# ToniChopp/ECAMP

Hardware: AMD Instinct MI355X
Metric: pretrain image-report pairs/sec (ViT-B/16, 224^2, seq=128) (higher is better)
Workload: dtype bf16

## Files before the change

ecamp_amd/csrc/core.hip:

```cpp
#include "common.h"
#include "attention.h"
#include "options.h"
#include "../../include/ecamp_hip.h"
#include <atomic>
#include <stdarg.h>
#include <stdlib.h>

thread_local char g_ecamp_err[512] = {0};

int ecamp_set_error(int code, const char* fmt, ...) {
    va_list ap;
    va_start(ap, fmt);
    vsnprintf(g_ecamp_err, sizeof(g_ecamp_err), fmt, ap);
    va_end(ap);
    return code;
}

extern "C" const char* ecamp_last_error(void) { return g_ecamp_err; }
extern "C" int ecamp_abi_version(void) { return ECAMP_ABI_VERSION; }
extern "C" int ecamp_half_format(void) { return ECAMP_HALF_IS_F16; }

#define OPT_UNREAD (INT_MIN + 1)
struct OptRow {
    const char* name; const char* env; int def; int (*set)(int);
    std::atomic<int> value{OPT_ENV};
    std::atomic<int> env_value{OPT_UNREAD};
};
static OptRow g_opts[OPT_COUNT] = {
              {"q8_mode", "ECAMP_GEMM_Q8", -1, [](int v) { return v == 0 || v == 2 ? v : -1; }},
               {"q8_sch", "ECAMP_Q8_SCH", 7, [](int v) { return v >= 0 ? v : OPT_ENV; }},
             {"q16_mode", "ECAMP_Q16", 1, [](int v) { return v >= 0 && v <= 3 ? v : OPT_ENV; }},
                {nullptr, "ECAMP_F8_Q8", 1, nullptr},
         {nullptr, "ECAMP_Q8_MIN_ITEMS", OPT_AUTO, nullptr},
          {"q8_bwd_grid", "ECAMP_Q8_BWD_GRID", 0, [](int v) { return v > 0 ? v : OPT_ENV; }},
             {"p8_wgrad", nullptr, 1, [](int v) { return v ? 1 : 0; }},
     {"p8_wgrad_reserve_cus", nullptr, 0, [](int v) { return v < 0 ? 0 : v; }},
          {nullptr, "ECAMP_WGRAD_ITEMS", 0, nullptr},
           {nullptr, "ECAMP_WGRAD_PLAN", 1, nullptr},
      {nullptr, "ECAMP_WGRAD_GROUP_CUS", 0, nullptr},
        {nullptr, "ECAMP_GEMM_GRID_CAP", 0, nullptr},
            {"attn_head", "ECAMP_ATTN_HEAD", 1, [](int v) { return v < 0 ? OPT_ENV : v ? 1 : 0; }},
           {nullptr, "ECAMP_ATTN_WAVES", 0, nullptr},
               {nullptr, "ECAMP_LN_BWD", 0, nullptr},
            {nullptr, "ECAMP_CE_KERNEL", 1, nullptr},
            {nullptr, "ECAMP_SR_BLOCKS", 512, nullptr},
};
int ecamp_opt_default(EcampOpt id) { return g_opts[id].def; }
int ecamp_opt(EcampOpt id) {
    OptRow& o = g_opts[id];
    const int s = o.value.load(std::memory_order_relaxed);
    if (s != OPT_ENV) return s;
    int e = o.env_value.load(std::memory_order_relaxed);
    if (e == OPT_UNREAD) {
        const char* txt = o.env ? getenv(o.env) : nullptr;
        e = txt ? atoi(txt) : o.def;
        o.env_value.store(e, std::memory_order_relaxed);
    }
    return e;
}
bool ecamp_opt_set(const char* name, int value) {
    for (OptRow& o : g_opts)
        if (o.name && strcmp(name, o.name) == 0) {
            o.value.store(o.set(value), std::memory_order_relaxed);
            return true;
        }
    return false;
}
extern "C" int ecamp_set_option(const char* name, int32_t value) {
    ECAMP_CHECK_ARG(name != nullptr, "set_option: null name");
    if (strcmp(name, "attn_head") == 0) { attn_set_head_mode(value); return 0; }
    if (ecamp_opt_set(name, value)) return 0;
    return ecamp_set_error(-1, "set_option: unknown option '%s'", name);
}

__global__ void dev_spin_kernel(long long cycles) {
    const long long t0 = clock64();
    while (clock64() - t0 < cycles) {}
}
extern "C" int ecamp_dev_spin(int32_t blocks, int32_t threads, int64_t cycles, hipStream_t stream) {
    ECAMP_CHECK_ARG(blocks > 0 && threads > 0 && threads <= 1024 && cycles >= 0, "dev_spin: bad arguments");
    hipLaunchKernelGGL(dev_spin_kernel, dim3(blocks), dim3(threads), 0, stream, (long long)cycles);
    ECAMP_LAUNCH_CHECK();
    return 0;
}
// ... 1 lines not shown
```

ecamp_amd/csrc/gemm.hip:

```cpp
#include "common.h"
#include <stdlib.h>
#include <string.h>
#include <stdint.h>
#include <map>
#include <string>
#include <vector>

#include "gemm_args.h"
#include "gemm_q8.h"
#include "gemm_q16.h"

#define BM 128
#define BN 128
#define BK 64

__device__ __forceinline__ int swz(int row) { return (row >> 1) & 7; }

__device__ __forceinline__ void g2r_kc(const bf16_t* P, long ld, int row0, int nrows, int k0, int kend, int tid,
                                       uint4 (&r)[4]) {
#pragma unroll
    for (int i = 0; i < 4; ++i) {
        int c = tid + 256 * i;
        int row = c >> 3, kc = c & 7;
        int gr = row0 + row, gk = k0 + kc * 8;
// ... 585 lines not shown
    if (g.out_f32) return (!g.bias && !g.residual && !g.pre_out && !g.gmul && !g.act) ? 4 : -1;
    if (g.gmul) return (!g.bias && !g.pre_out && (g.act == 0 || g.act == 2)) ? 3 : -1;
    if (g.pre_out || g.act) return (g.pre_out && (g.act == 1 || g.act == 2) && !g.residual) ? 1 : -1;
    if (g.residual) return 2;
    return 0;
}
static gemm_fn q8_pick(int a_kc, int b_kc, int epi, bool rowsum) {
    const int sch = ecamp_opt(OPT_Q8_SCH);
#define Q8S(A, B, E, R) ((gemm_fn)gemm_bf16_q8_kernel<A, B, E, 0, R, 1>)
    if (a_kc && b_kc && (sch & 1)) return epi == 0 ? Q8S(true, true, 0, false) : epi == 1 ? Q8S(true, true, 1, false) : epi == 2 ? Q8S(true, true, 2, false) :
                                          epi == 5 ? Q8S(true, true, 5, false) : (gemm_fn) nullptr;
    if (a_kc && !b_kc && (sch & 2)) return epi == 0 ? Q8S(true, false, 0, false) : epi == 2 ? Q8S(true, false, 2, false) : epi == 3 ? Q8S(true, false, 3, false) : (gemm_fn) nullptr;
    if (!a_kc && !b_kc && epi == 4 && (sch & 4)) return rowsum ? Q8S(false, false, 4, true) : Q8S(false, false, 4, false);
#undef Q8S
    if (a_kc && b_kc) return epi == 0 ? gemm_bf16_q8_kernel<true, true, 0> : epi == 1 ? gemm_bf16_q8_kernel<true, true, 1> : epi == 2 ? gemm_bf16_q8_kernel<true, true, 2> : (gemm_fn) nullptr;
    if (a_kc && !b_kc) return epi == 0 ? gemm_bf16_q8_kernel<true, false, 0> : epi == 2 ? gemm_bf16_q8_kernel<true, false, 2> : epi == 3 ? gemm_bf16_q8_kernel<true, false, 3> : (gemm_fn) nullptr;
    if (!a_kc && !b_kc && epi == 4) return rowsum ? gemm_bf16_q8_kernel<false, false, 4, 0, true> : gemm_bf16_q8_kernel<false, false, 4, 0, false>;
    return nullptr;
}
static bool q8_legal(const GemmArgs& g, int a_kc, int b_kc, int dtype, bool res32) {
    if (dtype != ECAMP_BF16) return false;
    const int epi = q8_epi(g, res32), split_k = g.nsplit;
    if (epi < 0 || !q8_pick(a_kc, b_kc, epi, g.rowsum != nullptr)) return false;
    if (split_k > 1 && epi != 4) return false;
    const long M = g.M, N = g.N, K = g.K;
    long kps = (K + split_k - 1) / split_k;
    kps = (kps + 63) / 64 * 64;
    const long ns = (K + kps - 1) / kps, last = K - (ns - 1) * kps;
    if (kps < 128 || last <= 64) return false;
    if (N % 8 || g.lda % 8 || g.ldb % 8 || !al16(g.A) || !al16(g.B) || !al16(g.C)) return false;
    if ((a_kc ? M * g.lda : K * g.lda) * 2 > LIM_2GB || (b_kc ? N * g.ldb : K * g.ldb) * 2 > LIM_2GB) return false;
    if (!a_kc && M % 8) return false;
    if (split_k > 1) { if (!al16(g.partial) || (long)split_k * M * N * 4 > LIM_2GB) return false; }
    else if (g.ldc % 8 || M * g.ldc * (epi >= 4 ? 4 : 2) > LIM_2GB) return false;
    if (g.bias && !al16(g.bias)) return false;
    if (g.pre_out && (g.ldp % 8 || !al16(g.pre_out) || M * g.ldp * 2 > LIM_2GB)) return false;
    if (g.gmul && (g.ldg % 8 || !al16(g.gmul) || M * g.ldg * 2 > LIM_2GB)) return false;
    if (g.residual && (g.ldr % 8 || !al16(g.residual) || M * g.ldr * (res32 ? 4 : 2) > LIM_2GB)) return false;
    return true;
}
static double q16_cost(int64_t M, int64_t N, int tn, int ncu) {
    const long tiles = (long)ceil_div(M, 256) * ceil_div(N, tn);
    return (double)((tiles + ncu - 1) / ncu) * (tn == 192 ? 0.79 : 1.0);
}
static gemm_fn q16_pick(int b_kc, int epi, int nw) {
    if (epi == 5) return b_kc ? (nw == 8 ? (gemm_fn)gemm_bf16_q16_kernel<5, 8, true> : (gemm_fn)gemm_bf16_q16_kernel<5, 6, true>) : (gemm_fn) nullptr;
    if (b_kc) {
        if (nw == 8) return epi == 0 ? (gemm_fn)gemm_bf16_q16_kernel<0, 8, true> : (gemm_fn)gemm_bf16_q16_kernel<2, 8, true>;
        return epi == 0 ? (gemm_fn)gemm_bf16_q16_kernel<0, 6, true> : (gemm_fn)gemm_bf16_q16_kernel<2, 6, true>;
    }
    if (nw == 8) return epi == 0 ? (gemm_fn)gemm_bf16_q16_kernel<0, 8, false> : (gemm_fn)gemm_bf16_q16_kernel<2, 8, false>;
    return epi == 0 ? (gemm_fn)gemm_bf16_q16_kernel<0, 6, false> : (gemm_fn)gemm_bf16_q16_kernel<2, 6, false>;
}

enum GemmFamily { GEMM_T128, GEMM_Q8, GEMM_Q16 };
struct GemmChoice {
    GemmFamily family;
    gemm_fn fn;
    int tm, tn;
    int block;
    long cap;
    const char* name;
    char form, epi, tail;
};
static GemmChoice gemm_select(const GemmArgs& g, int a_kc, int b_kc, int dtype, bool res32) {
    const char form = a_kc && b_kc ? 'f' : a_kc ? 'd' : 'w';
    GemmChoice c = {GEMM_T128, t128_pick(dtype, a_kc, b_kc, g.rowsum != nullptr, res32), BM, BN, 256, 0, "t128", form, '-', 's'};
    const int q8m = ecamp_opt(OPT_Q8_MODE), m16 = ecamp_opt(OPT_Q16_MODE);
    const long items8 = (long)ceil_div(g.M, 256) * ceil_div(g.N, 256) * g.nsplit;
    if (q8m == 0 || !(q8m == 2 || items8 >= q8_min_items() || m16 == 3) || !(a_kc || b_kc || ecamp_opt(OPT_P8_WGRAD)) || !q8_legal(g, a_kc, b_kc, dtype, res32))
        return c;
    const int epi = q8_epi(g, res32), ncu = p8_num_cu();
    c.epi = (char)('0' + epi);
    const int bwd_grid = a_kc && !b_kc ? ecamp_opt(OPT_Q8_BWD_GRID) : 0;
    if (m16 > 0 && a_kc && (epi == 0 || epi == 2 || epi == 5) && g.nsplit == 1 && !g.rowsum && (b_kc || g.ldb % 8 == 0)) {
        const double c256 = q16_cost(g.M, g.N, 256, ncu), c192 = q16_cost(g.M, g.N, 192, ncu);
        const int nw = c192 <= 0.9 * c256 ? 6 : 8;
        if (m16 >= 2 || nw == 6) {
            c.family = GEMM_Q16; c.fn = q16_pick(b_kc, epi, nw); c.tm = 256; c.tn = nw * 32; c.block = 256; c.name = "q16"; c.tail = 'w';
            c.cap = bwd_grid > 0 ? bwd_grid : ncu;
            return c;
        }
    }
    c.family = GEMM_Q8; c.fn = q8_pick(a_kc, b_kc, epi, g.rowsum != nullptr); c.tm = 256; c.tn = 256; c.block = 512; c.name = "q8";
    c.cap = bwd_grid > 0 ? bwd_grid : a_kc && b_kc ? ncu : p8_bwd_cus();
    return c;
}

extern "C" int ecamp_gemm_suggest_split(int64_t M, int64_t N, int64_t K, int a_kc, int b_kc, int dtype) {
    if (M <= 0 || N <= 0 || K <= 0) return 1;
    const int ncu = a_kc && b_kc ? p8_num_cu() : p8_bwd_cus();
    const long tiles = (long)ceil_div(M, 128) * ceil_div(N, 128);
    long s_old = 1024 / tiles;
    if (s_old < 1) s_old = 1;
    const long cap = (K + 255) / 256;
    if (s_old > cap) s_old = cap;
    if (dtype != ECAMP_BF16 || ecamp_opt(OPT_Q8_MODE) == 0 || (a_kc != 0) != (b_kc != 0) || (!a_kc && !b_kc && !ecamp_opt(OPT_P8_WGRAD))) return (int)s_old;
    const long t8 = (long)ceil_div(M, 256) * ceil_div(N, 256);
    const long tgt = (!a_kc && !b_kc) ? wgrad_target_items(ncu) : ncu;
    int best = 1;
    double best_score = -1.0;
    for (int sp = 1; sp <= 32; ++sp) {
        if (sp > 1 && K / sp < 512) break;
        const long items = t8 * sp;
        const long rounds = (items + tgt - 1) / tgt;
        const double score = (double)items / (double)(rounds * tgt) - 0.012 * (sp - 1);
        if (score > best_score + 1e-9) { best_score = score; best = sp; }
    }
    return t8 * best >= q8_min_items() ? best : (int)s_old;
}

extern "C" int64_t ecamp_gemm_workspace_bytes(int64_t M, int64_t N, int64_t K, int32_t split_k) {
    (void)K;
    return split_k > 1 && M > 0 && N > 0 ? (int64_t)split_k * M * N * 4 : 0;
}

static int gemm_call(const void* A, const void* B, void* C, int64_t M, int64_t N, int64_t K, int a_kc, int64_t lda,
                     int b_kc, int64_t ldb, int64_t ldc, const float* bias, const void* residual, int64_t ldr,
                     void* pre_out, int64_t ldp, const void* gmul, int64_t ldg, int act, float alpha, const float* alpha_dev, int dtype,
                     int out_f32, int accumulate, int split_k, float* splitk_ws, float* rowsum, hipStream_t stream, bool res32) {
    ECAMP_CHECK_ARG(A && B && C, "ecamp_gemm: null operand");
    ECAMP_CHECK_ARG(M > 0 && N > 0 && K > 0, "ecamp_gemm: bad shape %ld %ld %ld", (long)M, (long)N, (long)K);
    ECAMP_CHECK_ARG(dtype == ECAMP_F32 || dtype == ECAMP_BF16, "ecamp_gemm: bad dtype %d", dtype);
    ECAMP_CHECK_ARG(act >= 0 && act <= 2, "ecamp_gemm: act=%d (0 none, 1 GELU, 2 GELU with the saved derivative)", act);
    ECAMP_CHECK_ARG(act != 2 || (dtype == ECAMP_BF16 && !out_f32 && ((pre_out != nullptr) != (gmul != nullptr))),
                    "ecamp_gemm: act=2 (saved derivative) is the bf16 forward form with pre_out or the data-gradient form with gmul");
    const int vec = dtype == ECAMP_BF16 ? 8 : 4;
    const int ovec = dtype == ECAMP_BF16 ? 8 : 4;
    ECAMP_CHECK_ARG(N % 4 == 0, "ecamp_gemm: N=%ld must be a multiple of 4", (long)N);
    if (a_kc) ECAMP_CHECK_ARG(K % vec == 0 && lda % vec == 0, "ecamp_gemm: K/lda alignment (A k-contiguous)");
    else ECAMP_CHECK_ARG(M % ovec == 0 && lda % ovec == 0, "ecamp_gemm: M/lda alignment (A m-contiguous), M=%ld", (long)M);
    if (b_kc) ECAMP_CHECK_ARG(K % vec == 0 && ldb % vec == 0, "ecamp_gemm: K/ldb alignment (B k-contiguous)");
    else ECAMP_CHECK_ARG(N % ovec == 0 && ldb % ovec == 0, "ecamp_gemm: N/ldb alignment (B n-contiguous)");
    ECAMP_CHECK_ARG(!accumulate || out_f32 || dtype == ECAMP_F32, "ecamp_gemm: accumulate needs an f32 output");
    ECAMP_CHECK_ARG(!rowsum || (!a_kc && !b_kc), "ecamp_gemm: rowsum is built for the weight-gradient form (both operands strided) only");
// ... 261 lines not shown
extern "C" int64_t ecamp_wgrad_group_table_bytes(int32_t n, const int64_t* n_out, const int64_t* k_in, int64_t rows) {
    if (!ecamp_wgrad_group_supported(n, n_out, k_in, rows)) return 0;
    const long tiles = wg_tiles(n, n_out, k_in), ncu = p8_num_cu();
    return (tiles + ncu + 1) * (long)sizeof(Q8ItemRec) + ((ncu + 2) * 4 + 31) / 32 * 32 + tiles * (long)sizeof(WgTile) + 64;
}
extern "C" int64_t ecamp_wgrad_group_table(int32_t n, const int64_t* n_out, const int64_t* k_in, const int32_t* has_bias, int64_t rows,
                                           int32_t workgroups, void* host_table) {
    if (!n_out || !k_in || !has_bias || !host_table || !ecamp_wgrad_group_supported(n, n_out, k_in, rows))
        return ecamp_set_error(-1, "wgrad_group_table: unsupported group or null pointer");
    unsigned hb[4] = {0, 0, 0, 0};
    for (int p = 0; p < n; ++p) hb[p] = has_bias[p] ? 1u : 0u;
    const WgPlan* pl = wg_plan(n, n_out, k_in, hb, rows, ecamp_wgrad_group_workgroups(workgroups));
    char* out = (char*)host_table;
    memcpy(out, pl->items.data(), pl->items.size() * sizeof(Q8ItemRec));
    memcpy(out + pl->off_first, pl->first.data(), pl->first.size() * sizeof(int));
    memcpy(out + pl->off_tiles, pl->tiles.data(), pl->tiles.size() * sizeof(WgTile));
    return (int64_t)pl->bytes;
}
extern "C" int ecamp_wgrad_group(int32_t n, const void* const* dy, const void* const* x, float* const* gw, float* const* gb, const int64_t* n_out,
                                 const int64_t* k_in, int64_t rows, float alpha, const float* alpha_dev, const int32_t* accumulate, float* ws,
                                 const void* table, int64_t table_bytes, int32_t workgroups, hipStream_t stream) {
    ECAMP_CHECK_ARG(dy && x && gw && gb && n_out && k_in && accumulate && ws && table, "wgrad_group: null pointer");
    ECAMP_CHECK_ARG(((uintptr_t)table & 31) == 0, "wgrad_group: the item table must be 32-byte aligned");
    ECAMP_CHECK_ARG(ecamp_wgrad_group_supported(n, n_out, k_in, rows), "wgrad_group: unsupported group (1-4 layers, rows >= 256, dims %% 8 == 0, < 2 GB operands)");
    unsigned hb[4] = {0, 0, 0, 0};
    bool any_bias = false;
    for (int p = 0; p < n; ++p) {
        ECAMP_CHECK_ARG(dy[p] && x[p] && gw[p], "wgrad_group: null operand");
        ECAMP_CHECK_ARG(((uintptr_t)dy[p] & 15) == 0 && ((uintptr_t)x[p] & 15) == 0 && ((uintptr_t)gw[p] & 15) == 0, "wgrad_group: operands must be 16-byte aligned");
        hb[p] = gb[p] ? 1u : 0u;
        any_bias = any_bias || gb[p];
    }
    const int nwg = ecamp_wgrad_group_workgroups(workgroups);
    const WgPlan* pl = wg_plan(n, n_out, k_in, hb, rows, nwg);
    ECAMP_CHECK_ARG(table_bytes == (int64_t)pl->bytes, "wgrad_group: the item table (%ld bytes) was not built for the current plan (%ld bytes: CU reserve "
                    "or workgroup count changed since ecamp_wgrad_group_table) -- rebuild it", (long)table_bytes, (long)pl->bytes);
    const char* tb = (const char*)table;
    Q8Group G;
    memset(&G, 0, sizeof(G));
    G.items = (const Q8ItemRec*)tb; G.wg_first = (const int*)(tb + pl->off_first); G.slabs = ws; G.nprob = n;
    WgRedArgs R;
    memset(&R, 0, sizeof(R));
    R.tiles = (const WgTile*)(tb + pl->off_tiles); R.slabs = ws; R.ntiles = pl->ntiles;
    for (int p = 0; p < n; ++p) {
        G.p[p].A = dy[p]; G.p[p].B = x[p]; G.p[p].lda = n_out[p]; G.p[p].ldb = k_in[p]; G.p[p].M = (int)n_out[p]; G.p[p].N = (int)k_in[p];
        G.p[p].rowsum = gb[p]; G.p[p].alpha_out = alpha; G.p[p].alpha_dev_out = alpha_dev;
        R.p[p].C = gw[p]; R.p[p].ldc = k_in[p]; R.p[p].M = (int)n_out[p]; R.p[p].N = (int)k_in[p]; R.p[p].alpha = alpha; R.p[p].alpha_dev = alpha_dev;
        R.p[p].accumulate = accumulate[p];
    }
    GemmArgs g = gemm_args(dy[0], x[0], ws, n_out[0], k_in[0], rows, n_out[0], k_in[0], k_in[0]);
    g.out_f32 = 1; g.alpha_out = alpha; g.nbm = 1; g.nbn = 1; g.wide = 1; g.partial = ws;
    typedef void (*q8i_fn)(GemmArgs, Q8Group);
    const bool lean = (ecamp_opt(OPT_Q8_SCH) & 8) != 0;
    const q8i_fn fn = any_bias ? (lean ? (q8i_fn)gemm_bf16_q8_items_kernel<true, 1> : (q8i_fn)gemm_bf16_q8_items_kernel<true, 0>)
                               : (lean ? (q8i_fn)gemm_bf16_q8_items_kernel<false, 1> : (q8i_fn)gemm_bf16_q8_items_kernel<false, 0>);
    double work = 0.0;
    for (int p = 0; p < n; ++p) work += 2.0 * (double)n_out[p] * (double)k_in[p] * (double)rows;
    const bool prof = ecamp_prof_active();
    if (prof) {
        char tag[40];
        snprintf(tag, sizeof tag, "grp:w:n%d:%ld:%ld:%ld:wg%d", n, (long)rows, (long)n_out[0], (long)k_in[0], pl->nwg);
        ecamp_prof_begin(ECAMP_PROF_GEMM_BF16, work, stream, tag);
    }
    launch_persistent(fn, (long)pl->nwg, (long)pl->nwg, 512, stream, g, G);
    g_q8_launches += n;
    ++g_wg_launches;
    hipLaunchKernelGGL(wgrad_group_reduce_kernel, dim3(pl->ntiles * 16), dim3(256), 0, stream, R);
    if (prof) ecamp_prof_end(stream);
    ECAMP_LAUNCH_CHECK();
    return 0;
}
```

ecamp_amd/csrc/gemm_q16.h:

```cpp
#pragma once
#include "gemm_q8.h"

typedef __attribute__((ext_vector_type(4))) float q16_f32x4;

__device__ __forceinline__ int q16_key_m(int row) { return (row >> 1) & 7; }
__device__ __forceinline__ int q16_key_n(int row) { return ((row >> 1) & 1) | (((row >> 3) & 3) << 1); }

template <bool KC> struct Q16FragN;
template <> struct Q16FragN<true> {
    hw_bf16x8 v;
    __device__ __forceinline__ void read(const unsigned char* p, int off) { v = *reinterpret_cast<const hw_bf16x8*>(p + off); }
    __device__ __forceinline__ hw_bf16x8 get() const { return v; }
};
template <> struct Q16FragN<false> {
    q8_v4s16 lo, hi;
    template <int OFF> __device__ __forceinline__ void read_tr(const unsigned char* p) {
        const unsigned a = (unsigned)(size_t)(const __attribute__((address_space(3))) unsigned char*)p;
        asm volatile("ds_read_b64_tr_b16 %0, %1 offset:%2" : "=v"(lo) : "v"(a), "n"(OFF));
        asm volatile("ds_read_b64_tr_b16 %0, %1 offset:%2" : "=v"(hi) : "v"(a), "n"(OFF + 4 * 256));
    }
    __device__ __forceinline__ hw_bf16x8 get() const {
        return __builtin_bit_cast(hw_bf16x8, (bf16x8){lo[0], lo[1], lo[2], lo[3], hi[0], hi[1], hi[2], hi[3]});
    }
};
// ... 269 lines not shown
        Q16_KSTEP(1, false, 0, 0, sMn, sNn, 2, 3);                                                                       \
        rA = Q16_RS(rA, 2); rB = Q16_RS(rB, 2);                                                                          \
    } while (0)

    q_cv(false);
    if (qv < total) Q16_ITEM();
    Q16_ISSUE_ALL(0); Q16_ADVANCE(0); Q16_ISSUE_ALL(1); Q16_ADVANCE(1); Q16_ISSUE_ALL(2); Q16_ADVANCE(2); Q16_ISSUE_ALL(3); Q16_ADVANCE(3);
    Q16_ISSUE_ALL(0); Q16_ADVANCE(0); Q16_ISSUE_ALL(1); Q16_ADVANCE(1); Q16_ISSUE_ALL(2); Q16_ADVANCE(2); Q16_ISSUE_ALL(3); Q16_ADVANCE(3);
    if (NPB == 4) asm volatile("s_waitcnt vmcnt(16)" ::: "memory"); else asm volatile("s_waitcnt vmcnt(14)" ::: "memory");
    __builtin_amdgcn_s_barrier();
    {
        const unsigned char* sM = lds + wr * Q8_HALF;
        const unsigned char* sN = lds + (NSLOT + wc) * Q8_HALF;
        Q16_RDB(0, 0, 0, sN); Q16_RDB(0, 0, 1, sN); Q16_RDB(0, 0, 2, sN); Q16_RDB(0, 0, 3, sN); Q16_RDB(0, 0, 4, sN); Q16_RDB(0, 0, 5, sN);
        if (NW == 8) { Q16_RDB(0, 0, (NW == 8 ? 6 : 0), sN); Q16_RDB(0, 0, (NW == 8 ? 7 : 0), sN); }
        Q16_RDA(0, 0, 0, sM); Q16_RDA(0, 0, 1, sM); Q16_RDA(0, 0, 2, sM); Q16_RDA(0, 0, 3, sM);
        Q16_RDA(0, 0, 4, sM); Q16_RDA(0, 0, 5, sM); Q16_RDA(0, 0, 6, sM); Q16_RDA(0, 0, 7, sM);
    }

    for (int cv = it_beg; cv < total; cv += G) {
        int cm0, cn0;
        decode(cv, cm0, cn0);
        bias_request(cn0);
        Q16_KTILE(true);
        bias_landed();
#pragma unroll 1
        for (int t = 1; t < nt; ++t) Q16_KTILE(false);
        Q16_WAIT_SET(0);
        Q16_STORE_TILE(cm0, cn0);
    }
    asm volatile("s_waitcnt vmcnt(0)" ::: "memory");
#undef Q16_RS
#undef Q16_ITEM
#undef Q16_ISSUE1
#undef Q16_ISSUE_ALL
#undef Q16_ADVANCE
#undef Q16_STORE_TILE
#undef Q16_SB
#undef Q16_RDA
#undef Q16_RDB
#undef Q16_WAIT_SET
#undef Q16_MFMA
#undef Q16_SLOT
#undef Q16_PAIR
#undef Q16_PAIR4
#undef Q16_KSTEP
#undef Q16_KTILE
}

template <int EPI, int NW, bool B_KC, int DBG = 0>
__global__ __launch_bounds__(256) void gemm_bf16_q16_kernel(GemmArgs g) {
    q16_body<EPI, NW, B_KC, DBG>(g);
}
```

ecamp_amd/csrc/options.h:

```cpp
#pragma once
#include <limits.h>

enum EcampOpt {
    OPT_Q8_MODE, OPT_Q8_SCH, OPT_Q16_MODE, OPT_F8_Q8, OPT_Q8_MIN_ITEMS, OPT_Q8_BWD_GRID, OPT_P8_WGRAD, OPT_P8_WGRAD_RESERVE,
    OPT_WGRAD_ITEMS, OPT_WGRAD_PLAN, OPT_WGRAD_GROUP_CUS, OPT_GEMM_GRID_CAP, OPT_ATTN_HEAD, OPT_ATTN_WAVES, OPT_LN_BWD, OPT_CE_KERNEL,
    OPT_SR_BLOCKS, OPT_COUNT
};
#define OPT_ENV INT_MIN
#define OPT_AUTO INT_MIN

#define ECAMP_HIDDEN __attribute__((visibility("hidden")))
ECAMP_HIDDEN int ecamp_opt(EcampOpt id);
ECAMP_HIDDEN int ecamp_opt_default(EcampOpt id);
ECAMP_HIDDEN bool ecamp_opt_set(const char* name, int value);
```

Before: 7122.

## Add 4-wave q16 weight-gradient GEMM kernel for layer and grouped wgrad

Adds a new 256-thread (4-wave) weight-gradient GEMM kernel built on the q16 design. It uses a 5-slot LDS ring with buffer-load-to-LDS prefetch and a 256x256 tile per block, and comes in both per-layer and grouped persistent-item variants. By default it replaces the 512-thread q8 items kernel for grouped wgrad, and also the q8 path for large layer wgrad with epilogue 4. The goal is higher MFMA utilisation and better scheduling in the backward weight-gradient GEMMs. The risks are register pressure from the 8x8 accumulator tile held by fewer waves, and correctness issues in the hand-scheduled pipeline.

```diff
diff --git a/ecamp_amd/csrc/core.hip b/ecamp_amd/csrc/core.hip
--- a/ecamp_amd/csrc/core.hip
+++ b/ecamp_amd/csrc/core.hip
@@ -30,6 +30,7 @@
               {"q8_mode", "ECAMP_GEMM_Q8", -1, [](int v) { return v == 0 || v == 2 ? v : -1; }},
                {"q8_sch", "ECAMP_Q8_SCH", 7, [](int v) { return v >= 0 ? v : OPT_ENV; }},
              {"q16_mode", "ECAMP_Q16", 1, [](int v) { return v >= 0 && v <= 3 ? v : OPT_ENV; }},
+            {"q16_wgrad", "ECAMP_Q16_WGRAD", 1, [](int v) { return v >= 0 && v <= 2 ? v : OPT_ENV; }},
                 {nullptr, "ECAMP_F8_Q8", 1, nullptr},
          {nullptr, "ECAMP_Q8_MIN_ITEMS", OPT_AUTO, nullptr},
           {"q8_bwd_grid", "ECAMP_Q8_BWD_GRID", 0, [](int v) { return v > 0 ? v : OPT_ENV; }},
diff --git a/ecamp_amd/csrc/gemm.hip b/ecamp_amd/csrc/gemm.hip
--- a/ecamp_amd/csrc/gemm.hip
+++ b/ecamp_amd/csrc/gemm.hip
@@ -661,6 +661,14 @@
     if (nw == 8) return epi == 0 ? (gemm_fn)gemm_bf16_q16_kernel<0, 8, false> : (gemm_fn)gemm_bf16_q16_kernel<2, 8, false>;
     return epi == 0 ? (gemm_fn)gemm_bf16_q16_kernel<0, 6, false> : (gemm_fn)gemm_bf16_q16_kernel<2, 6, false>;
 }
+enum Q16WgradClass { Q16W_GROUPED = 1, Q16W_LAYER = 2 };
+static bool q16_wgrad_on(int cls, const GemmArgs* g = nullptr) {
+    const int m = ecamp_opt(OPT_Q16_WGRAD);
+    if (m >= 2) return true;
+    if (m != 1 || ecamp_opt(OPT_Q16_MODE) == 0) return false;
+    if (cls == Q16W_GROUPED) return true;
+    return g && g->M >= 256 && g->N >= 256 && (long)ceil_div(g->M, 256) * ceil_div(g->N, 256) * g->nsplit >= q8_min_items();
+}
 
 enum GemmFamily { GEMM_T128, GEMM_Q8, GEMM_Q16 };
 struct GemmChoice {
@@ -677,7 +685,8 @@
     GemmChoice c = {GEMM_T128, t128_pick(dtype, a_kc, b_kc, g.rowsum != nullptr, res32), BM, BN, 256, 0, "t128", form, '-', 's'};
     const int q8m = ecamp_opt(OPT_Q8_MODE), m16 = ecamp_opt(OPT_Q16_MODE);
     const long items8 = (long)ceil_div(g.M, 256) * ceil_div(g.N, 256) * g.nsplit;
-    if (q8m == 0 || !(q8m == 2 || items8 >= q8_min_items() || m16 == 3) || !(a_kc || b_kc || ecamp_opt(OPT_P8_WGRAD)) || !q8_legal(g, a_kc, b_kc, dtype, res32))
+    const bool w16 = !a_kc && !b_kc && ecamp_opt(OPT_Q16_WGRAD) == 2;
+    if (q8m == 0 || !(q8m == 2 || items8 >= q8_min_items() || m16 == 3 || w16) || !(a_kc || b_kc || ecamp_opt(OPT_P8_WGRAD)) || !q8_legal(g, a_kc, b_kc, dtype, res32))
         return c;
     const int epi = q8_epi(g, res32), ncu = p8_num_cu();
     c.epi = (char)('0' + epi);
@@ -690,6 +699,11 @@
             c.cap = bwd_grid > 0 ? bwd_grid : ncu;
             return c;
         }
+    }
+    if (!a_kc && !b_kc && epi == 4 && q16_wgrad_on(Q16W_LAYER, &g)) {
+        c.family = GEMM_Q16; c.fn = g.rowsum ? (gemm_fn)gemm_bf16_q16_wgrad_kernel<true> : (gemm_fn)gemm_bf16_q16_wgrad_kernel<false>;
+        c.tm = 256; c.tn = 256; c.block = 256; c.name = "q16"; c.cap = p8_bwd_cus();
+        return c;
     }
     c.family = GEMM_Q8; c.fn = q8_pick(a_kc, b_kc, epi, g.rowsum != nullptr); c.tm = 256; c.tn = 256; c.block = 512; c.name = "q8";
     c.cap = bwd_grid > 0 ? bwd_grid : a_kc && b_kc ? ncu : p8_bwd_cus();
@@ -1057,18 +1071,21 @@
     g.out_f32 = 1; g.alpha_out = alpha; g.nbm = 1; g.nbn = 1; g.wide = 1; g.partial = ws;
     typedef void (*q8i_fn)(GemmArgs, Q8Group);
     const bool lean = (ecamp_opt(OPT_Q8_SCH) & 8) != 0;
-    const q8i_fn fn = any_bias ? (lean ? (q8i_fn)gemm_bf16_q8_items_kernel<true, 1> : (q8i_fn)gemm_bf16_q8_items_kernel<true, 0>)
+    const bool four = q16_wgrad_on(Q16W_GROUPED);
+    const q8i_fn fn = four ? (any_bias ? (q8i_fn)gemm_bf16_q16_wgrad_items_kernel<true> : (q8i_fn)gemm_bf16_q16_wgrad_items_kernel<false>)
+                    : any_bias ? (lean ? (q8i_fn)gemm_bf16_q8_items_kernel<true, 1> : (q8i_fn)gemm_bf16_q8_items_kernel<true, 0>)
                                : (lean ? (q8i_fn)gemm_bf16_q8_items_kernel<false, 1> : (q8i_fn)gemm_bf16_q8_items_kernel<false, 0>);
     double work = 0.0;
     for (int p = 0; p < n; ++p) work += 2.0 * (double)n_out[p] * (double)k_in[p] * (double)rows;
     const bool prof = ecamp_prof_active();
     if (prof) {
         char tag[40];
-        snprintf(tag, sizeof tag, "grp:w:n%d:%ld:%ld:%ld:wg%d", n, (long)rows, (long)n_out[0], (long)k_in[0], pl->nwg);
+        snprintf(tag, sizeof tag, "%s:w:n%d:%ld:%ld:%ld:wg%d", four ? "grp16" : "grp", n, (long)rows, (long)n_out[0], (long)k_in[0], pl->nwg);
         ecamp_prof_begin(ECAMP_PROF_GEMM_BF16, work, stream, tag);
     }
-    launch_persistent(fn, (long)pl->nwg, (long)pl->nwg, 512, stream, g, G);
+    launch_persistent(fn, (long)pl->nwg, (long)pl->nwg, four ? 256 : 512, stream, g, G);
     g_q8_launches += n;
+    if (four) ++g_q16_launches;
     ++g_wg_launches;
     hipLaunchKernelGGL(wgrad_group_reduce_kernel, dim3(pl->ntiles * 16), dim3(256), 0, stream, R);
     if (prof) ecamp_prof_end(stream);
diff --git a/ecamp_amd/csrc/gemm_q16.h b/ecamp_amd/csrc/gemm_q16.h
--- a/ecamp_amd/csrc/gemm_q16.h
+++ b/ecamp_amd/csrc/gemm_q16.h
@@ -345,3 +345,338 @@
 __global__ __launch_bounds__(256) void gemm_bf16_q16_kernel(GemmArgs g) {
     q16_body<EPI, NW, B_KC, DBG>(g);
 }
+
+template <bool ROWSUM, bool ITEMS>
+__device__ __forceinline__ void q16w_body(const GemmArgs& g, const Q8Group& GR) {
+    constexpr int NSLOT = 5, NW = 8;
+    extern __shared__ __attribute__((aligned(16))) unsigned char lds[];
+    const int tid = threadIdx.x, lane = tid & 63, wave = __builtin_amdgcn_readfirstlane(tid >> 6);
+    const int wr = wave >> 1, wc = wave & 1;
+    const int l15 = lane & 15, lq = lane >> 4;
+    typedef const int __attribute__((address_space(4))) cint4;
+    const int it_beg = ITEMS ? *(cint4*)(GR.wg_first + blockIdx.x) : (int)blockIdx.x;
+    const int total = ITEMS ? *(cint4*)(GR.wg_first + blockIdx.x + 1) : g.nbm * g.nbn * g.nsplit, G = ITEMS ? 1 : (int)gridDim.x;
+    typedef int q16_i32x8 __attribute__((ext_vector_type(8)));
+    typedef const q16_i32x8 __attribute__((address_space(4))) crec4;
+    static_assert(sizeof(Q8Prob) == 64 && offsetof(Q8Prob, A) == 0 && offsetof(Q8Prob, B) == 8 && offsetof(Q8Prob, lda) == 16 && offsetof(Q8Prob, ldb) == 24 &&
+                  offsetof(Q8Prob, M) == 32 && offsetof(Q8Prob, rowsum) == 40 && offsetof(Q8Prob, alpha_dev_out) == 48 && offsetof(Q8Prob, alpha_out) == 56 &&
+                  alignof(Q8Group) == 8, "q16w_body reads Q8Prob as two 32-byte records");
+    const unsigned char __attribute__((address_space(4)))* const probs =
+        (const unsigned char __attribute__((address_space(4)))*)__builtin_amdgcn_kernarg_segment_ptr() + ((sizeof(GemmArgs) + 7) & ~(size_t)7) + offsetof(Q8Group, p);
+    auto prob_half = [&](int prob, int half) { return *(crec4*)(probs + prob * 64 + half * 32); };
+    auto ptr_of = [](int lo, int hi) {
+        return (const void*)(((unsigned long long)(unsigned)__builtin_amdgcn_readfirstlane(hi) << 32) | (unsigned)__builtin_amdgcn_readfirstlane(lo));
+    };
+    float* const gr_slabs = GR.slabs;
+    auto item_at = [&](int i) {
+        const q16_i32x8 w = *(crec4*)(reinterpret_cast<const int*>(GR.items) + (long)i * 8);
+        Q8ItemRec r;
+#define Q16W_U(X) __builtin_amdgcn_readfirstlane(X)
+        r.prob = Q16W_U(w[0]); r.m0 = Q16W_U(w[1]); r.n0 = Q16W_U(w[2]); r.kbeg = Q16W_U(w[3]); r.kend = Q16W_U(w[4]); r.slab = Q16W_U(w[5]); r.flags = Q16W_U(w[6]); r.pad = 0;
+#undef Q16W_U
+        return r;
+    };
+    auto uniform_ptr = [](const void* q) {
+        const unsigned long long v = (unsigned long long)q;
+        const unsigned lo = (unsigned)__builtin_amdgcn_readfirstlane((int)(unsigned)v), hi = (unsigned)__builtin_amdgcn_readfirstlane((int)(unsigned)(v >> 32));
+        return (const void*)(((unsigned long long)hi << 32) | lo);
+    };
+
+    unsigned offM[4], offN[4];
+    {
+        const int r = l15 >> 2, q = l15 & 3;
+#pragma unroll
+        for (int T = 0; T < 4; ++T) {
+            offM[T] = (unsigned)((8 * lq + r) * 256 + ((((T ^ r) << 2) | (q >> 1)) << 4) + (q & 1) * 8);
+            offN[T] = (unsigned)((8 * lq + r) * 256 + ((((4 * T + q) ^ (r << 2)) & 15) << 4));
+        }
+    }
+    q16_f32x4 acc[8][NW];
+
+    const unsigned char *qa = reinterpret_cast<const unsigned char*>(g.A), *qb = reinterpret_cast<const unsigned char*>(g.B);
+    int qa_rec = 0, qb_rec = 0, q_krem = 1 << 30, qv = it_beg;
+    int a_step = (int)g.lda * 128, b_step = (int)g.ldb * 128;
+    long q_lda = ITEMS ? -1 : g.lda, q_ldb = ITEMS ? -1 : g.ldb;
+    unsigned cvA[8], cvB[8];
+    int dA = wave * 4096, dB = NSLOT * Q8_HALF + wave * 4096;
+    auto q_cv = [&]() __attribute__((always_inline)) {
+#pragma unroll
+        for (int j = 0; j < 4; ++j) {
+            const int kr = (wave * 4 + j) * 4 + (lane >> 4);
+            const int oc = (lane & 15) ^ ((kr & 3) << 2);
+            cvA[j] = (unsigned)(((long)kr * q_lda + oc * 8) * 2); cvA[4 + j] = cvA[j] + 256u;
+            cvB[j] = (unsigned)(((long)kr * q_ldb + oc * 8) * 2); cvB[4 + j] = cvB[j] + 256u;
+        }
+    };
+#define Q16W_ITEM()                                                                                                      \
+    do {                                                                                                                 \
+        if (ITEMS) {                                                                                                     \
+            const Q8ItemRec r_ = item_at(qv);                                                                            \
+            const q16_i32x8 p_ = prob_half(r_.prob, 0);                                                                  \
+            const long la_ = __builtin_amdgcn_readfirstlane(p_[4]), lb_ = __builtin_amdgcn_readfirstlane(p_[6]);    \
+            const unsigned char* A_ = reinterpret_cast<const unsigned char*>(ptr_of(p_[0], p_[1]));                      \
+            const unsigned char* B_ = reinterpret_cast<const unsigned char*>(ptr_of(p_[2], p_[3]));                      \
+            q_krem = r_.kend - r_.kbeg;                                                                                  \
+            qa = A_ + ((long)r_.kbeg * la_ + r_.m0) * 2; qa_rec = (int)(((long)q_krem * la_ - r_.m0) * 2);               \
+            qb = B_ + ((long)r_.kbeg * lb_ + r_.n0) * 2; qb_rec = (int)(((long)q_krem * lb_ - r_.n0) * 2);               \
+            a_step = (int)la_ * 128; b_step = (int)lb_ * 128;                                                            \
+            if (la_ != q_lda || lb_ != q_ldb) { q_lda = la_; q_ldb = lb_; q_cv(); }                                      \
+        } else {                                                                                                         \
+            const Q8Item n_ = q8_decode<6>(g, qv, total);                                                                \
+            q_krem = n_.kend - n_.kbeg;                                                                                  \
+            qa = reinterpret_cast<const unsigned char*>(g.A) + ((long)n_.kbeg * g.lda + n_.m0) * 2; qa_rec = (int)(((long)q_krem * g.lda - n_.m0) * 2); \
+            qb = reinterpret_cast<const unsigned char*>(g.B) + ((long)n_.kbeg * g.ldb + n_.n0) * 2; qb_rec = (int)(((long)q_krem * g.ldb - n_.n0) * 2); \
+        }                                                                                                                \
+        qa_rec = max(qa_rec, 0); qb_rec = max(qb_rec, 0);                                                                \
+    } while (0)
+    typedef void __attribute__((address_space(3))) lds_void_;
+#define Q16W_ISSUE1(PART, J)                                                                                             \
+    do {                                                                                                                 \
+        constexpr bool isA_ = (((PART) & 1) == 0);                                                                       \
+        constexpr int h_ = (PART) >> 1;                                                                                  \
+        const __amdgpu_buffer_rsrc_t rs_ = __builtin_amdgcn_make_buffer_rsrc((void*)(isA_ ? qa : qb), 0, isA_ ? qa_rec : qb_rec, 0x00020000); \
+        unsigned char* d_ = lds + (isA_ ? dA : dB) + (J) * 1024;                                                         \
+        __builtin_amdgcn_raw_ptr_buffer_load_lds(rs_, (lds_void_*)d_, 16, (int)(isA_ ? cvA[4 * h_ + (J)] : cvB[4 * h_ + (J)]), 0, 0, 0); \
+    } while (0)
+#define Q16W_ADVANCE(PART)                                                                                               \
+    do {                                                                                                                 \
+        if (((PART) & 1) == 0) { dA += Q8_HALF; if (dA >= NSLOT * Q8_HALF) dA -= NSLOT * Q8_HALF; }                      \
+        else                   { dB += Q8_HALF; if (dB >= 2 * NSLOT * Q8_HALF) dB -= NSLOT * Q8_HALF; }                  \
+        if ((PART) == 3) {                                                                                               \
+            q_krem -= 64;                                                                                                \
+            qa += a_step; qb += b_step; qa_rec = max(qa_rec - a_step, 0); qb_rec = max(qb_rec - b_step, 0);              \
+            if (q_krem <= 0) {                                                                                           \
+                qv += G;                                                                                                 \
+                if (qv < total) Q16W_ITEM(); else { qa_rec = 0; qb_rec = 0; q_krem = 1 << 30; }                          \
+            }                                                                                                            \
+        }                                                                                                                \
+    } while (0)
+#define Q16W_ISSUE_ALL(PART) do { Q16W_ISSUE1(PART, 0); Q16W_ISSUE1(PART, 1); Q16W_ISSUE1(PART, 2); Q16W_ISSUE1(PART, 3); } while (0)
+#define Q16W_SB() __builtin_amdgcn_sched_barrier(0)
+
+    float rs[8];
+    const unsigned rs_ones = H16_ONE_X2;
+    typedef unsigned q16_u32x2 __attribute__((ext_vector_type(2)));
+
+    const unsigned lane_slab = (unsigned)(((wr * 128 + l15) * 256 + wc * 128 + 8 * lq) * 4);
+    auto store_block = [&](int pm0, int pn0, int pz, auto p_c) __attribute__((always_inline)) {
+        constexpr int P = decltype(p_c)::value;
+        typedef const float __attribute__((address_space(4))) cfloat4;
+        unsigned uo[8];
+        int so[8];
+        float al = 1.f;
+        bool accum = false;
+        __amdgpu_buffer_rsrc_t rO;
+        if constexpr (ITEMS) {
+            rO = __builtin_amdgcn_make_buffer_rsrc((void*)uniform_ptr(gr_slabs + (long)pz * 65536), 0, 262144, 0x00020000);
+#pragma unroll
+            for (int I = 0; I < 8; ++I) { uo[I] = lane_slab; so[I] = (I * 16 * 256 + P * 32) * 4; }
+        } else {
+            const int nb = pn0 + wc * 128 + P * 32 + 8 * lq;
+            const bool oob = nb >= g.N;
+            if (g.partial) {
+                rO = __builtin_amdgcn_make_buffer_rsrc((void*)g.partial, 0, (int)(unsigned)((long)g.nsplit * g.M * g.N * 4), 0x00020000);
+#pragma unroll
+                for (int I = 0; I < 8; ++I) {
+                    const int row = pm0 + wr * 128 + I * 16 + l15;
+                    uo[I] = (oob || row >= g.M) ? 0x80000000u : (unsigned)((((long)pz * g.M + row) * g.N + nb) * 4);
+                    so[I] = 0;
+                }
+            } else {
+                rO = __builtin_amdgcn_make_buffer_rsrc(g.C, 0, (int)(unsigned)((long)g.M * g.ldc * 4), 0x00020000);
+                al = g.alpha;
+                if (g.alpha_dev) { float ad = *(cfloat4*)g.alpha_dev; asm volatile("" : "+s"(ad)); al *= ad; }
+                accum = g.accumulate != 0;
+#pragma unroll
+                for (int I = 0; I < 8; ++I) {
+                    const int row = pm0 + wr * 128 + I * 16 + l15;
+                    uo[I] = oob ? 0x80000000u : (unsigned)(((long)row * g.ldc + nb) * 4);
+                    so[I] = 0;
+                }
+            }
+        }
+        q8_u32x4 qo[8], qo2[8];
+        if (!ITEMS && accum) {
+#pragma unroll
+            for (int I = 0; I < 8; ++I) {
+                qo[I] = __builtin_amdgcn_raw_buffer_load_b128(rO, uo[I], 0, 0);
+                qo2[I] = __builtin_amdgcn_raw_buffer_load_b128(rO, uo[I] + 16, 0, 0);
+            }
+        }
+        Q16W_SB();
+#pragma unroll
+        for (int I = 0; I < 8; ++I) {
+            float v[8];
+#pragma unroll
+            for (int r = 0; r < 4; ++r) {
+                float x0, x1;
+                asm volatile("v_accvgpr_read_b32 %0, %1" : "=v"(x0) : "a"(acc[I][2 * P][r]));
+                asm volatile("v_accvgpr_read_b32 %0, %1" : "=v"(x1) : "a"(acc[I][2 * P + 1][r]));
+                v[r] = ITEMS ? x0 : x0 * al; v[4 + r] = ITEMS ? x1 : x1 * al;
+            }
+            if (!ITEMS && accum) {
+#pragma unroll
+                for (int r = 0; r < 4; ++r) { v[r] += __uint_as_float(qo[I][r]); v[4 + r] += __uint_as_float(qo2[I][r]); }
+            }
+            __builtin_amdgcn_raw_buffer_store_b128((q8_u32x4){__float_as_uint(v[0]), __float_as_uint(v[1]), __float_as_uint(v[2]), __float_as_uint(v[3])}, rO, uo[I], so[I], 0);
+            __builtin_amdgcn_raw_buffer_store_b128((q8_u32x4){__float_as_uint(v[4]), __float_as_uint(v[5]), __float_as_uint(v[6]), __float_as_uint(v[7])}, rO, uo[I] + 16, so[I], 0);
+            Q16W_SB();
+        }
+    };
+    auto rowsum_flush = [&](int pm0, float al, const float* adp, float* dst, int dstM) __attribute__((always_inline)) {
+        typedef const float __attribute__((address_space(4))) cfloat4;
+        if (adp) { float ad = *(cfloat4*)adp; asm volatile("" : "+s"(ad)); al *= ad; }
+        const __amdgpu_buffer_rsrc_t rS = __builtin_amdgcn_make_buffer_rsrc((void*)dst, 0, (int)(unsigned)((long)dstM * 4), 0x00020000);
+#pragma unroll
+        for (int I = 0; I < 8; ++I) {
+            float tot = rs[I] + __shfl_xor(rs[I], 16, 64);
+            tot = (tot + __shfl_xor(tot, 32, 64)) * al;
+            const unsigned off = lq ? 0x80000000u : (unsigned)((pm0 + wr * 128 + I * 16 + l15) * 4);
+            __builtin_amdgcn_raw_ptr_buffer_atomic_fadd_f32(tot, rS, off, 0, 0);
+        }
+    };
+    const q16_f32x4 zero4 = {0.f, 0.f, 0.f, 0.f};
+
+    Q16FragN<false> fa[2][8], fb[2][NW];
+#define Q16W_RDA(S, KS, I, SM_) fa[S][I].template read_tr<((I) & 1) * 32 + (KS) * 8192>((SM_) + offM[(I) >> 1])
+#define Q16W_RDB(S, KS, T, SN_) fb[S][T].template read_tr<((T) & 1) * 8 + (KS) * 8192>((SN_) + offN[(T) >> 1])
+    auto wait_set = [&](Q16FragN<false> (&f)[8], Q16FragN<false> (&e)[8]) __attribute__((always_inline)) {
+        asm volatile("s_waitcnt lgkmcnt(0)" : "+v"(f[0].lo), "+v"(f[0].hi), "+v"(f[1].lo), "+v"(f[1].hi), "+v"(f[2].lo), "+v"(f[2].hi), "+v"(f[3].lo), "+v"(f[3].hi),
+                     "+v"(f[4].lo), "+v"(f[4].hi), "+v"(f[5].lo), "+v"(f[5].hi), "+v"(f[6].lo), "+v"(f[6].hi), "+v"(f[7].lo), "+v"(f[7].hi));
+        asm volatile("" : "+v"(e[0].lo), "+v"(e[0].hi), "+v"(e[1].lo), "+v"(e[1].hi), "+v"(e[2].lo), "+v"(e[2].hi), "+v"(e[3].lo), "+v"(e[3].hi),
+                     "+v"(e[4].lo), "+v"(e[4].hi), "+v"(e[5].lo), "+v"(e[5].hi), "+v"(e[6].lo), "+v"(e[6].hi), "+v"(e[7].lo), "+v"(e[7].hi));
+    };
+#define Q16W_WAIT_SET(S) do { wait_set(fb[S], fa[S]); Q16W_SB(); } while (0)
+#define Q16W_MFMA(S, J, ZERO)                                                                                            \
+    do {                                                                                                                 \
+        constexpr int i_ = (J) / NW, t_ = (J) % NW;                                                                      \
+        acc[i_][t_] = ECAMP_MFMA_16x16x32(fb[S][t_].get(), fa[S][i_].get(), (ZERO) ? zero4 : acc[i_][t_]);               \
+    } while (0)
+#define Q16W_RS(S, s_, ON)                                                                                               \
+    do {                                                                                                                 \
+        if constexpr (ROWSUM && (ON)) {                                                                                        \
+            constexpr int i_ = (s_) >> 2, j_ = (s_) & 3;                                                                 \
+            const unsigned w_ = j_ < 2 ? __builtin_bit_cast(q16_u32x2, fa[S][i_].lo)[j_ & 1] : __builtin_bit_cast(q16_u32x2, fa[S][i_].hi)[j_ & 1]; \
+            asm(ECAMP_DOT2C " %0, %1, %2" : "+v"(rs[i_]) : "v"(w_), "v"(rs_ones));                                       \
+        }                                                                                                                \
+    } while (0)
+#define Q16W_SLOT(NS, NKS, SM_, SN_, DP0, DP1, s_)                                                                       \
+    do {                                                                                                                 \
+        constexpr int s__ = (s_);                                                                                        \
+        if (s__ < 8) Q16W_RDB(NS, NKS, (s__ < 8 ? s__ : 0), SN_);                                                        \
+        else if (s__ < 16) Q16W_RDA(NS, NKS, (s__ >= 8 && s__ < 16 ? s__ - 8 : 0), SM_);                                 \
+        else if (s__ < 20) { Q16W_ISSUE1(DP0, (s__ - 16) & 3); }                                                         \
+        else if (s__ == 20) { Q16W_ADVANCE(DP0); }                                                                       \
+        else if (s__ < 25) { Q16W_ISSUE1(DP1, (s__ - 21) & 3); }                                                         \
+        else if (s__ == 25) { Q16W_ADVANCE(DP1); }                                                                       \
+    } while (0)
+#define Q16W_PAIR(S, ZERO, NS, NKS, SM_, SN_, DP0, DP1, RS_, s_)                                                         \
+    do {                                                                                                                 \
+        Q16W_MFMA(S, 2 * (s_), ZERO); Q16W_MFMA(S, 2 * (s_) + 1, ZERO); Q16W_RS(S, s_, RS_); Q16W_SB();                  \
+        Q16W_SLOT(NS, NKS, SM_, SN_, DP0, DP1, s_); Q16W_SB();                                                           \
+    } while (0)
+#define Q16W_PAIR4(S, Z, NS, NKS, SM_, SN_, D0, D1, s_) \
+    do { Q16W_PAIR(S, Z, NS, NKS, SM_, SN_, D0, D1, RS_, (s_)); Q16W_PAIR(S, Z, NS, NKS, SM_, SN_, D0, D1, RS_, (s_) + 1); Q16W_PAIR(S, Z, NS, NKS, SM_, SN_, D0, D1, RS_, (s_) + 2); Q16W_PAIR(S, Z, NS, NKS, SM_, SN_, D0, D1, RS_, (s_) + 3); } while (0)
+#define Q16W_KSTEP(S, Z, NS, NKS, SM_, SN_, D0, D1, RSK_)                                                                    \
+    do {                                                                                                                 \
+        constexpr bool RS_ = (RSK_);                                                                                     \
+        Q16W_SB();                                                                                                       \
+        Q16W_WAIT_SET(S);                                                                                                \
+        Q16W_PAIR4(S, Z, NS, NKS, SM_, SN_, D0, D1, 0);  Q16W_PAIR4(S, Z, NS, NKS, SM_, SN_, D0, D1, 4);                 \
+        Q16W_PAIR4(S, Z, NS, NKS, SM_, SN_, D0, D1, 8);  Q16W_PAIR4(S, Z, NS, NKS, SM_, SN_, D0, D1, 12);                \
+        Q16W_PAIR4(S, Z, NS, NKS, SM_, SN_, D0, D1, 16); Q16W_PAIR4(S, Z, NS, NKS, SM_, SN_, D0, D1, 20);                \
+        Q16W_PAIR4(S, Z, NS, NKS, SM_, SN_, D0, D1, 24); Q16W_PAIR4(S, Z, NS, NKS, SM_, SN_, D0, D1, 28);                \
+    } while (0)
+    int rA = 0, rB = 0;
+#define Q16W_RS_(R_, ADD_) ((R_) + (ADD_) >= NSLOT ? (R_) + (ADD_) - NSLOT : (R_) + (ADD_))
+#define Q16W_KTILE(FIRST, RSV)                                                                                             \
+    do {                                                                                                                 \
+        const unsigned char* sM = lds + Q16W_RS_(rA, wr) * Q8_HALF;                                                      \
+        const unsigned char* sN = lds + (NSLOT + Q16W_RS_(rB, wc)) * Q8_HALF;                                            \
+        const unsigned char* sMn = lds + Q16W_RS_(rA, 2 + wr) * Q8_HALF;                                                 \
+        const unsigned char* sNn = lds + (NSLOT + Q16W_RS_(rB, 2 + wc)) * Q8_HALF;                                       \
+        Q16W_KSTEP(0, FIRST, 1, 1, sM, sN, 0, 1, (RSV) == 1);                                                            \
+        asm volatile("s_waitcnt vmcnt(8)" ::: "memory");                                                                 \
+        asm volatile("s_waitcnt lgkmcnt(0)" ::: "memory"); Q16W_SB();                                                    \
+        __builtin_amdgcn_s_barrier(); Q16W_SB();                                                                         \
+        Q16W_KSTEP(1, false, 0, 0, sMn, sNn, 2, 3, (RSV) == 2);                                                          \
+        rA = Q16W_RS_(rA, 2); rB = Q16W_RS_(rB, 2);                                                                      \
+    } while (0)
+
+    if (!ITEMS) q_cv();
+    if (qv < total) Q16W_ITEM();
+    Q16W_ISSUE_ALL(0); Q16W_ADVANCE(0); Q16W_ISSUE_ALL(1); Q16W_ADVANCE(1); Q16W_ISSUE_ALL(2); Q16W_ADVANCE(2); Q16W_ISSUE_ALL(3); Q16W_ADVANCE(3);
+    Q16W_ISSUE_ALL(0); Q16W_ADVANCE(0); Q16W_ISSUE_ALL(1); Q16W_ADVANCE(1); Q16W_ISSUE_ALL(2); Q16W_ADVANCE(2); Q16W_ISSUE_ALL(3); Q16W_ADVANCE(3);
+    asm volatile("s_waitcnt vmcnt(16)" ::: "memory");
+    __builtin_amdgcn_s_barrier();
+    {
+        const unsigned char* sM = lds + wr * Q8_HALF;
+        const unsigned char* sN = lds + (NSLOT + wc) * Q8_HALF;
+        Q16W_RDB(0, 0, 0, sN); Q16W_RDB(0, 0, 1, sN); Q16W_RDB(0, 0, 2, sN); Q16W_RDB(0, 0, 3, sN);
+        Q16W_RDB(0, 0, 4, sN); Q16W_RDB(0, 0, 5, sN); Q16W_RDB(0, 0, 6, sN); Q16W_RDB(0, 0, 7, sN);
+        Q16W_RDA(0, 0, 0, sM); Q16W_RDA(0, 0, 1, sM); Q16W_RDA(0, 0, 2, sM); Q16W_RDA(0, 0, 3, sM);
+        Q16W_RDA(0, 0, 4, sM); Q16W_RDA(0, 0, 5, sM); Q16W_RDA(0, 0, 6, sM); Q16W_RDA(0, 0, 7, sM);
+    }
+    Q16W_WAIT_SET(0);
+
+    for (int cv = it_beg; cv < total; cv += G) {
+        int cm0, cn0, cz, cnt, cprob = 0;
+        bool rs_on = false;
+        if (ITEMS) {
+            const Q8ItemRec cr = item_at(cv);
+            cm0 = cr.m0; cn0 = cr.n0; cz = cr.slab; cprob = cr.prob; cnt = (cr.kend - cr.kbeg + 63) >> 6;
+            if (ROWSUM) { const q16_i32x8 p_ = prob_half(cr.prob, 1); rs_on = (cr.flags & 1) != 0 && (p_[2] | p_[3]) != 0; }
+        } else {
+            const Q8Item cit = q8_decode<6>(g, cv, total);
+            cm0 = cit.m0; cn0 = cit.n0; cz = cit.z; cnt = cit.nt;
+            if (ROWSUM) rs_on = g.rowsum != nullptr && cit.ncol == 0;
+        }
+#define Q16W_KLOOP(RSV) do { Q16W_KTILE(true, RSV); _Pragma("unroll 1") for (int t = 1; t < cnt; ++t) Q16W_KTILE(false, RSV); Q16W_WAIT_SET(0); } while (0)
+        if (ROWSUM && rs_on) {
+#pragma unroll
+            for (int I = 0; I < 8; ++I) rs[I] = 0.f;
+            if (wc == 0) Q16W_KLOOP(1); else Q16W_KLOOP(2);
+        } else {
+            Q16W_KLOOP(0);
+        }
+#undef Q16W_KLOOP
+        if (ROWSUM) {
+            if (rs_on) {
+                if (ITEMS) {
+                    const q16_i32x8 p_ = prob_half(cprob, 1);
+                    rowsum_flush(cm0, __int_as_float(__builtin_amdgcn_readfirstlane(p_[6])), (const float*)ptr_of(p_[4], p_[5]), (float*)ptr_of(p_[2], p_[3]),
+                                 __builtin_amdgcn_readfirstlane(p_[0]));
+                } else rowsum_flush(cm0, g.alpha_out, g.alpha_dev_out, g.rowsum, g.M);
+            }
+        }
+        store_block(cm0, cn0, cz, std::integral_constant<int, 0>()); store_block(cm0, cn0, cz, std::integral_constant<int, 1>());
+        store_block(cm0, cn0, cz, std::integral_constant<int, 2>()); store_block(cm0, cn0, cz, std::integral_constant<int, 3>());
+    }
+    asm volatile("s_waitcnt vmcnt(0)" ::: "memory");
+#undef Q16W_ITEM
+#undef Q16W_ISSUE1
+#undef Q16W_ISSUE_ALL
+#undef Q16W_ADVANCE
+#undef Q16W_SB
+#undef Q16W_RDA
+#undef Q16W_RDB
+#undef Q16W_WAIT_SET
+#undef Q16W_MFMA
+#undef Q16W_RS
+#undef Q16W_SLOT
+#undef Q16W_PAIR
+#undef Q16W_PAIR4
+#undef Q16W_KSTEP
+#undef Q16W_RS_
+#undef Q16W_KTILE
+}
+
+template <bool ROWSUM>
+__global__ __launch_bounds__(256) void gemm_bf16_q16_wgrad_kernel(GemmArgs g) {
+    Q8Group none;
+    q16w_body<ROWSUM, false>(g, none);
+}
+template <bool ROWSUM>
+__global__ __launch_bounds__(256) void gemm_bf16_q16_wgrad_items_kernel(GemmArgs g, Q8Group GR) {
+    q16w_body<ROWSUM, true>(g, GR);
+}
diff --git a/ecamp_amd/csrc/options.h b/ecamp_amd/csrc/options.h
--- a/ecamp_amd/csrc/options.h
+++ b/ecamp_amd/csrc/options.h
@@ -2,7 +2,7 @@
 #include <limits.h>
 
 enum EcampOpt {
-    OPT_Q8_MODE, OPT_Q8_SCH, OPT_Q16_MODE, OPT_F8_Q8, OPT_Q8_MIN_ITEMS, OPT_Q8_BWD_GRID, OPT_P8_WGRAD, OPT_P8_WGRAD_RESERVE,
+    OPT_Q8_MODE, OPT_Q8_SCH, OPT_Q16_MODE, OPT_Q16_WGRAD, OPT_F8_Q8, OPT_Q8_MIN_ITEMS, OPT_Q8_BWD_GRID, OPT_P8_WGRAD, OPT_P8_WGRAD_RESERVE,
     OPT_WGRAD_ITEMS, OPT_WGRAD_PLAN, OPT_WGRAD_GROUP_CUS, OPT_GEMM_GRID_CAP, OPT_ATTN_HEAD, OPT_ATTN_WAVES, OPT_LN_BWD, OPT_CE_KERNEL,
     OPT_SR_BLOCKS, OPT_COUNT
 };
```

Result: faster. 7253 (median of 6 runs) (+1.8%).
